# jiexray/gelly-streaming

Measured on AMD Instinct MI355X. Metric: edges/sec (whole node) for streaming CC on RMAT-26, higher is better.
Workload: dtype int64; 1 GPU; rmat26-cc-stream; scale=26, edges=1073741824, micro_batch=1048576, combine_every_edges_per_gpu=4194304, combine=none at 1 GPU (same cadence), ids=sparse 64-bit (scrambled), capacity_hint=33554432, vertices_labelled=32802821, parallelism=single GPU

## Files before the change

gelly-streaming_amd/__init__.py:

```python
import ctypes
import os

import numpy as np


_HERE = os.path.dirname(os.path.abspath(__file__))
LIB_PATH = os.path.join(_HERE, "lib", "libgs_summary.so")
if os.environ.get("GS_LIB_VARIANT"):
    LIB_PATH = os.path.join(_HERE, "lib_" + os.environ["GS_LIB_VARIANT"], "libgs_summary.so")

KIND_CC = 0
KIND_SIGNED = 1
KIND_DEGREE = 2

DEGREE_ALL = 0
DEGREE_IN = 1
DEGREE_OUT = 2

GS_OK = 0
GS_ERR_INVALID = -1
GS_ERR_HIP = -2
GS_ERR_CAPACITY = -3
GS_ERR_TRUNCATED = -4
GS_ERR_PARSE = -5

SEP_WHITESPACE = 0
SEP_TAB = 1

KERNEL_IDS = {"fold": 0, "stage": 1, "export": 2, "init": 3}

EXPORTED_SYMBOLS = (
    "gs_last_error", "gs_version", "gs_create", "gs_destroy", "gs_reset", "gs_fold", "gs_fold_device",
    "gs_combine", "gs_sync", "gs_num_vertices", "gs_find", "gs_export_labels", "gs_export_labels_device",
    "gs_bip_status", "gs_export_colouring", "gs_serialize", "gs_deserialize", "gs_set_delta_tracking",
    "gs_take_delta_records", "gs_fold_take_device", "gs_delta_stage", "gs_fold_records_device", "gs_fold_exchange_device",
    "gs_get_stream", "gs_set_pipelining", "gs_set_hot_index", "gs_hot_index_stats", "gs_set_profiling", "gs_kernel_stats", "gs_table_capacity", "gs_counters", "gs_debug_counters",
    "gs_gen_rmat", "gs_gen_er", "gs_gen_bip",
    "gs_parse_edges_device", "gs_fold_text", "gs_parse_set_profiling", "gs_parse_profile", "gs_parse_release",
    "gs_group_unique_id", "gs_group_create", "gs_group_fold_device", "gs_group_finish", "gs_group_stats",
    "gs_group_destroy", "gs_group_tree_combine", "gs_combine_exported_device",
    "gs_group_fold_batches_device", "gs_group_set_ramp", "gs_export_labels_part_device",
    "gs_delta_capacity", "gs_find_labels_device", "gs_capacity_stats",
    "gs_set_change_tracking", "gs_take_changes_device", "gs_take_changes",
    "gs_fold_records_counted_device", "gs_reset_config", "gs_wait_event", "gs_wait_stream", "gs_fold_device_after",
    "gs_fold_parity", "gs_set_window_server", "gs_window_server_stats", "gs_set_batch_dedup",
    "gs_digest", "gs_group_comm_ranks", "gs_group_set_phase_timing", "gs_group_phase_stats",
    "gs_group_set_comm_api", "gs_testing_set", "gs_testing_get", "gs_testing_group_forest", "gs_hbm_bytes", "gs_create_bytes",
    "gs_group_create_partitioned", "gs_group_part_fold_device", "gs_group_part_combine",
    "gs_group_part_labels_device", "gs_group_part_status", "gs_group_part_reset", "gs_group_part_stats",
    "gs_group_part_phase_stats",
    "gs_num_components", "gs_export_components_device", "gs_export_components",
    "gs_degree_fold", "gs_degree_fold_device", "gs_degree_find_device", "gs_degree_export_device",
    "gs_degree_export", "gs_degree_distribution_device", "gs_degree_distribution",
    "gs_triangle_create", "gs_triangle_destroy", "gs_triangle_reset", "gs_triangle_fold", "gs_triangle_fold_device",
    "gs_triangle_count", "gs_triangle_count_device", "gs_triangle_find_device", "gs_triangle_export_device",
    "gs_triangle_export", "gs_triangle_sync", "gs_triangle_get_stream", "gs_triangle_wait_stream",
    "gs_testing_triangle_stats", "gs_testing_triangle_bins",
    "gs_slice_create", "gs_slice_destroy", "gs_slice_window", "gs_slice_window_device", "gs_slice_size",
    "gs_slice_reduce_device", "gs_slice_reduce", "gs_slice_neighborhoods_device", "gs_slice_neighborhoods",
    "gs_slice_sync", "gs_slice_get_stream", "gs_slice_wait_stream", "gs_testing_slice_stats",
    "gs_distinct_create", "gs_distinct_destroy", "gs_distinct_reset", "gs_distinct_fold", "gs_distinct_fold_device",
    "gs_distinct_size", "gs_distinct_new_edges_device", "gs_distinct_new_edges", "gs_distinct_new_vertices_device",
    "gs_distinct_new_vertices", "gs_distinct_vertices_device", "gs_distinct_vertices", "gs_distinct_edges_device",
    "gs_distinct_edges", "gs_distinct_rank_device", "gs_distinct_contains_device", "gs_distinct_sync",
    "gs_distinct_get_stream", "gs_distinct_wait_stream", "gs_testing_distinct_stats",
    "gs_testing_distinct_phases",
    "gs_spanner_create", "gs_spanner_destroy", "gs_spanner_reset", "gs_spanner_fold", "gs_spanner_fold_device",
    "gs_spanner_add", "gs_spanner_within", "gs_spanner_within_device", "gs_spanner_combine", "gs_spanner_count",
    "gs_spanner_export_device", "gs_spanner_export", "gs_spanner_neighbors", "gs_spanner_sync",
# ... 122 lines not shown
    L.gs_window_server_stats.argtypes = [_vp, ctypes.POINTER(_u64), ctypes.POINTER(_u64)]
    L.gs_fold_device.argtypes = [_vp, _vp, _vp, _vp, _sz, _sz]
    L.gs_fold_device_after.argtypes = [_vp, _vp, _vp, _vp, _sz, _sz, _vp]
    L.gs_wait_event.argtypes = [_vp, _vp]
    L.gs_wait_stream.argtypes = [_vp, _vp]
    L.gs_combine.argtypes = [_vp, _vp]
    L.gs_sync.argtypes = [_vp]
    L.gs_num_vertices.argtypes = [_vp, ctypes.POINTER(_u64)]
    L.gs_find.argtypes = [_vp, _i64, ctypes.POINTER(_i64), ctypes.POINTER(ctypes.c_int)]
    L.gs_export_labels.argtypes = [_vp, _vp, _vp, _sz, ctypes.POINTER(_sz)]
    L.gs_export_labels_device.argtypes = [_vp, _vp, _vp, _vp, _sz, ctypes.POINTER(_sz)]
    L.gs_bip_status.argtypes = [_vp, ctypes.POINTER(ctypes.c_int)]
    L.gs_export_colouring.argtypes = [_vp, _vp, _vp, _vp, _sz, ctypes.POINTER(_sz)]
    L.gs_serialize.argtypes = [_vp, _vp, _sz, ctypes.POINTER(_sz)]
    L.gs_deserialize.argtypes = [_vp, _vp, _sz]
    L.gs_set_delta_tracking.argtypes = [_vp, ctypes.c_int]
    L.gs_take_delta_records.argtypes = [_vp, _vp, _sz, _vp]
    L.gs_fold_take_device.argtypes = [_vp, _vp, _vp, _sz, _vp, _sz, _vp, _vp]
    L.gs_fold_records_device.argtypes = [_vp, _vp, _sz, ctypes.c_int]
    L.gs_fold_records_counted_device.argtypes = [_vp, _vp, _sz, _vp, ctypes.c_int]
    L.gs_delta_stage.argtypes = [_vp, _vp, _sz, ctypes.c_int, _vp]
    L.gs_fold_exchange_device.argtypes = [_vp, _vp, _vp, _sz, _sz, ctypes.c_int, ctypes.c_int]
    L.gs_delta_capacity.argtypes = [_vp, ctypes.POINTER(_u64)]
    L.gs_find_labels_device.argtypes = [_vp, _vp, _sz, _vp, _vp]
    L.gs_capacity_stats.argtypes = [_vp, ctypes.POINTER(_u64), ctypes.POINTER(_u64), ctypes.POINTER(ctypes.c_double)]
    L.gs_set_change_tracking.argtypes = [_vp, ctypes.c_int]
    L.gs_take_changes_device.argtypes = [_vp, _vp, _vp, _vp, _sz, ctypes.POINTER(_u64)]
    L.gs_take_changes.argtypes = [_vp, _vp, _vp, _vp, _sz, ctypes.POINTER(_u64)]
    L.gs_get_stream.argtypes = [_vp, ctypes.POINTER(_vp)]
    L.gs_set_profiling.argtypes = [_vp, ctypes.c_int]
    L.gs_set_pipelining.argtypes = [_vp, ctypes.c_int]
    L.gs_set_hot_index.argtypes = [_vp, ctypes.c_int, _u64, ctypes.c_uint32]
    L.gs_hot_index_stats.argtypes = [_vp, ctypes.POINTER(_u64)]
    L.gs_kernel_stats.argtypes = [_vp, ctypes.c_int, ctypes.POINTER(_u64), ctypes.POINTER(ctypes.c_double)]
    L.gs_table_capacity.argtypes = [_vp, ctypes.POINTER(_u64)]
    L.gs_counters.argtypes = [_vp, ctypes.POINTER(_u64)]
    L.gs_debug_counters.argtypes = [_vp, ctypes.POINTER(_u64), ctypes.c_int]
    L.gs_gen_rmat.argtypes = [_vp, _vp, _vp, _u64, _u64, ctypes.c_int, _u64, ctypes.c_int]
    L.gs_gen_er.argtypes = [_vp, _vp, _vp, _u64, _u64, ctypes.c_int, _u64, ctypes.c_int]
    L.gs_gen_bip.argtypes = [_vp, _vp, _vp, _u64, _u64, ctypes.c_int, _u64, _vp, _sz]
    L.gs_parse_edges_device.argtypes = [_vp, _vp, _sz, ctypes.c_int, _vp, _vp, _sz, ctypes.POINTER(_u64),
                                        ctypes.POINTER(_i64)]
    L.gs_parse_set_profiling.argtypes = [ctypes.c_int]
    L.gs_parse_profile.argtypes = [ctypes.POINTER(ctypes.c_double), ctypes.POINTER(_u64)]
    L.gs_fold_text.argtypes = [_vp, ctypes.c_char_p, _sz, ctypes.c_int, ctypes.POINTER(_u64), ctypes.POINTER(_i64)]
    L.gs_group_unique_id.argtypes = [_vp]
    L.gs_group_create.argtypes = [ctypes.POINTER(_vp), _vp, _vp, ctypes.c_int, ctypes.c_int, _sz]
    L.gs_group_fold_device.argtypes = [_vp, _vp, _vp, _sz]
    L.gs_group_finish.argtypes = [_vp]
    L.gs_group_stats.argtypes = [_vp, ctypes.POINTER(_u64), ctypes.POINTER(_u64), ctypes.POINTER(_u64)]
    L.gs_group_destroy.argtypes = [_vp]
    L.gs_group_tree_combine.argtypes = [_vp]
    L.gs_group_fold_batches_device.argtypes = [_vp, _vp, _vp, _sz, _sz]
    L.gs_group_set_ramp.argtypes = [_vp, _sz, _sz]
    L.gs_export_labels_part_device.argtypes = [_vp, ctypes.c_int, ctypes.c_int, _vp, _vp, _vp, _sz,
                                               ctypes.POINTER(_sz)]
    L.gs_combine_exported_device.argtypes = [_vp, _vp, _vp, _vp, _sz, ctypes.c_int]
    L.gs_digest.argtypes = [_vp, ctypes.POINTER(_u64)]
    L.gs_group_comm_ranks.argtypes = [_vp, ctypes.POINTER(ctypes.c_int), ctypes.POINTER(ctypes.c_int)]
    L.gs_group_set_phase_timing.argtypes = [_vp, ctypes.c_int]
    L.gs_group_phase_stats.argtypes = [_vp, ctypes.POINTER(ctypes.c_double)]
    L.gs_group_set_comm_api.argtypes = [_vp]
    L.gs_group_create_partitioned.argtypes = [ctypes.POINTER(_vp), _vp, _vp, ctypes.c_int, ctypes.c_int, _u64, _sz]
    L.gs_group_part_fold_device.argtypes = [_vp, _vp, _vp, _sz]
    L.gs_group_part_combine.argtypes = [_vp]
    L.gs_group_part_labels_device.argtypes = [_vp, _vp, _vp, _vp, _sz, ctypes.POINTER(_sz)]
# ... 170 lines not shown


def digest_rows(v, label, parity=None):
    import torch

    def srl(x, k):
        return (x >> k) & ((1 << (64 - k)) - 1)

    def mix(z):
        z = (z ^ srl(z, 30)) * -4658895280553007687
        z = (z ^ srl(z, 27)) * -7723592293110705685
        return z ^ srl(z, 31)
    if v.numel() == 0:
        return 0
    a = mix(v ^ 0x243F6A8885A308D3)
    b = mix(label + (parity.to(torch.int64) * 0x13198A2E03707344 if parity is not None else 0))
    return int(torch.sum(a * b).item()) & ((1 << 64) - 1)


TESTING_KNOBS = {"server_idle_us": 0, "changes_walk_max": 1, "parse_lb_timeout_us": 2, "group_self_apply": 3,
                 "group_data_lag": 4, "degree_variant": 5, "triangle_variant": 6, "triangle_profile": 7,
                 "slice_profile": 8, "distinct_profile": 9, "spanner_round_cap": 10, "spanner_lds_set": 11,
                 "spanner_arenas": 12}


def testing_set(knob, value):
    _check(lib().gs_testing_set(TESTING_KNOBS[knob], -1 if value is None else int(value)))


def testing_get(knob):
    return lib().gs_testing_get(TESTING_KNOBS[knob])


class testing:

    def __init__(self, **knobs):
        self.knobs = knobs

    def __enter__(self):
        for k, v in self.knobs.items():
            testing_set(k, v)
        return self

    def __exit__(self, *a):
        for k in self.knobs:
            testing_set(k, None)


FAKE_COMM_PATH = os.path.join(_HERE, "host", "bin", "libgs_fakecomm.so")
_fake = None


def fake_comm():
    global _fake
    if _fake is None:
        lib()
        if not os.path.exists(FAKE_COMM_PATH):
            raise ImportError("libgs_fakecomm.so not built (%s); run __graft_entry__.build()" % FAKE_COMM_PATH)
        F = ctypes.CDLL(FAKE_COMM_PATH)
        F.gs_fake_comm_api.restype = _vp
        F.gs_fake_comm_last_error.restype = ctypes.c_int
        F.gs_fake_comm_order_hash.restype = _u64
        _fake = F
    return _fake


# ... 1409 lines not shown
```

gelly-streaming_amd/csrc/gs_capi.cpp:

```cpp
#include <hip/hip_runtime.h>

#include <algorithm>
#include <atomic>
#include <chrono>
#include <mutex>
#include <unordered_map>
#include <cstdio>
#include <cstring>
#include <string>
#include <thread>
#include <vector>

#include "gs_ingest.h"
#include "gs_internal.hpp"

#ifndef GS_YOUNG_HEAD_LOG2
#define GS_YOUNG_HEAD_LOG2 14
#endif

namespace gsi {

thread_local std::string g_err;

int fail(int code, const std::string& msg) {
// ... 92 lines not shown
  if (h->x_v) {
    if (int rc = wait_x_consumer(h)) return rc;
    GS_HIP(hipStreamSynchronize(h->stream));
  }
  h->x_cap = 0;
  const uint64_t c = std::max<uint64_t>(rows, (uint64_t)(kMaxLoad * (double)h->cap) + 2);
  GS_HIP(h->x_v.alloc(c));
  GS_HIP(h->x_l.alloc(c));
  GS_HIP(h->x_p.alloc(c));
  h->x_cap = c;
  return GS_OK;
}

void reset_capacity_tracking(gs_summary* h, uint64_t nv) {
  h->rep_epoch++;
  h->nv_ub = nv;
  h->nv_exact = nv;
  h->e_exact = 0;
  h->e_launched = 0;
  h->e_lost = 0;
  for (int i = 0; i < gs_summary::kRepStreams; ++i) h->rep_skip[i] = 0, h->rep_pending[i] = 0;
  h->rep_pending_edges = 0;
}

#ifndef GS_HOT_LOG2
#define GS_HOT_LOG2 17
#endif
#ifndef GS_HOT_REFRESH_EVERY
#define GS_HOT_REFRESH_EVERY 16
#endif
#ifndef GS_HOT_SAMPLE_LOG2
#define GS_HOT_SAMPLE_LOG2 20
#endif
constexpr int kHotLog2 = GS_HOT_LOG2;
constexpr int kHotMaxLog2 = 20;
constexpr uint64_t kHotFirstEdges = 1ull << 26;
constexpr uint32_t kHotEvery = 2048;
constexpr uint32_t kHotRefreshEvery = GS_HOT_REFRESH_EVERY;
constexpr uint32_t kHotRefreshPerBuild = 16;
constexpr uint64_t kHotMinTableBytes = 256ull << 20;
constexpr size_t kHotSampleEdges = 1u << GS_HOT_SAMPLE_LOG2;

int hot_log2(const gs_summary* h) {
  if (h->kind != GS_KIND_CC || h->hot_cfg < 0) return 0;
  if (h->track || h->changes || h->srv_on || h->side || h->group_lanes) return 0;
  if (h->hot_cfg > 0) return h->hot_cfg;
  if (h->cap * sizeof(gs::Slot) < kHotMinTableBytes) return 0;
  return kHotLog2;
}

void hot_drop(gs_summary* h) {
  h->hot_live = -1;
  h->hot_building = -1;
  h->hot_read_on[0] = h->hot_read_on[1] = false;
  h->hot_edges = 0;
  h->hot_folds = 0;
  h->hot_folds_r = 0;
}

int hot_before_fold(gs_summary* h) {
  if (h->hot_building < 0 || hipEventQuery(h->hot_built) != hipSuccess) return GS_OK;
  const int old = h->hot_live;
  h->hot_live = h->hot_building;
  h->hot_building = -1;
  if (old < 0) return GS_OK;
  for (int i = 0; i <= gs_summary::kLanes; ++i) {
    hipStream_t st = i < gs_summary::kLanes ? (hipStream_t)h->lane[i] : (hipStream_t)h->stream;
    if (i < gs_summary::kLanes && !h->lane[i]) continue;
    GS_HIP(hipEventRecord(h->hot_read[old][i], st));
  }
  h->hot_read_on[old] = true;
  return GS_OK;
}

int hot_after_fold(gs_summary* h, const int64_t* src, const int64_t* dst, size_t c, size_t stride, hipStream_t st,
                   int hl) {
  h->hot_edges += c;
  h->hot_folds++;
  h->hot_folds_r++;
  if (h->hot_building >= 0) return GS_OK;
  const uint64_t first = h->hot_cfg ? h->hot_first : kHotFirstEdges;
  const uint32_t every = h->hot_cfg ? h->hot_every : kHotEvery;
  const bool build = h->hot_live < 0 ? h->hot_edges >= first : h->hot_folds >= every;
  const uint32_t refresh_every = h->hot_cfg ? every / kHotRefreshPerBuild : kHotRefreshEvery;
  if (!build) {
    if (!(h->hot_live >= 0 && refresh_every && h->hot_folds_r >= refresh_every)) return GS_OK;
    h->hot_refreshes++;
    h->hot_folds_r = 0;
    GS_LAUNCH(gs::launch_hot_refresh(h->table(), h->hot_buf[h->hot_live], hl, st));
    return GS_OK;
  }
  if (h->hot_alloc_log2 != hl) {
    h->hot_alloc_log2 = 0;
    for (auto& b : h->hot_buf) GS_HIP(b.alloc(gs::hot_buckets(hl) + 1));
    GS_HIP(h->hot_scratch.alloc(gs::hot_scratch_words(hl)));
    if (!h->hot_built) {
      GS_HIP(h->hot_built.create());
      for (auto& r : h->hot_read)
        for (Event& e : r) GS_HIP(e.create());
    }
    h->hot_alloc_log2 = hl;
  }
  const int b = h->hot_live < 0 ? 0 : h->hot_live ^ 1;
  if (h->hot_read_on[b]) {
    for (int i = 0; i <= gs_summary::kLanes; ++i)
      if (i == gs_summary::kLanes || h->lane[i]) GS_HIP(hipStreamWaitEvent(st, h->hot_read[b][i], 0));
    h->hot_read_on[b] = false;
  }
  h->hot_folds = 0;
  h->hot_builds++;
  GS_LAUNCH(gs::launch_hot_build(h->table(), src, dst, (uint32_t)std::min(c, kHotSampleEdges), (uint32_t)stride,
                                 h->hot_buf[b], hl, h->hot_scratch, st));
  GS_HIP(hipEventRecord(h->hot_built, st));
  h->hot_building = b;
  h->hot_folds_r = 0;
  return GS_OK;
}

}

uint64_t create_capacity(uint64_t capacity_hint) {
  const uint64_t cap = next_pow2(std::max<uint64_t>(kSlotsPerHintedVertex * std::max<uint64_t>(capacity_hint, 1), 1024));
  return std::min(cap, kMaxCap);
}

uint64_t create_bytes(uint64_t cap) {
  return (cap + 1) * sizeof(gs::Slot) + (uint64_t)gs::kShards * (cap / gs::kShards + 1024) * 4 +
         (uint64_t)gs::CTR_COUNT * gs::kCtrStride * 4 + 64;
}

namespace {

int alloc_vlist(gs_summary* h) {
  h->vshard_cap = (uint32_t)(h->cap / gs::kShards + 1024);
  GS_HIP(h->vlist.alloc((uint64_t)gs::kShards * h->vshard_cap));
  return GS_OK;
}

int alloc_table(gs_summary* h, uint64_t cap, bool keep_delta = false) {
  h->cap = cap;
  h->logcap = log2_ceil(cap);
  GS_HIP(h->tab.alloc(cap + 1));
  if (int rc = alloc_vlist(h)) return rc;
  memset(h->h_flags, 0, 16);
  hot_drop(h);
// ... 1507 lines not shown
  if (int rc = join_lanes(h)) return rc;
  GS_HIP(hipStreamSynchronize(h->stream));
  hot_drop(h);
  if (h->hot_alloc_log2 != (log2_entries > 0 ? log2_entries : kHotLog2)) {
    h->hot_alloc_log2 = 0;
    for (auto& b : h->hot_buf) b.reset();
    h->hot_scratch.reset();
  }
  h->hot_cfg = log2_entries < 0 ? -1 : log2_entries;
  h->hot_first = first_after_edges;
  h->hot_every = rebuild_every_folds;
  return GS_OK;
}

int gs_hot_index_stats(gs_handle h, uint64_t* out4) {
  if (int rc = check_any(h)) return rc;
  if (!out4) return fail(GS_ERR_INVALID, "out is null");
  DeviceGuard g(h->device);
  if (int rc = join_lanes(h)) return rc;
  GS_HIP(hipStreamSynchronize(h->stream));
  if (int rc = hot_before_fold(h)) return rc;
  out4[0] = h->hot_builds;
  out4[1] = 0;
  out4[2] = h->hot_live >= 0 ? (uint64_t)h->hot_alloc_log2 : 0;
  out4[3] = h->hot_refreshes;
  if (h->hot_live >= 0) {
    std::vector<gs::HotBucket> e(gs::hot_buckets(h->hot_alloc_log2));
    GS_HIP(hipMemcpy(e.data(), h->hot_buf[h->hot_live], e.size() * sizeof(gs::HotBucket), hipMemcpyDeviceToHost));
    for (const gs::HotBucket& x : e) out4[1] += (x.key[0] != gs::kEmpty) + (x.key[1] != gs::kEmpty);
  }
  return GS_OK;
}

int gs_table_capacity(gs_handle h, uint64_t* slots) {
  if (int rc = check_any(h)) return rc;
  if (!slots) return fail(GS_ERR_INVALID, "slots is null");
  *slots = h->cap;
  return GS_OK;
}

}

namespace gsi {

int x_scratch(gs_summary* h, uint64_t rows) {
  if (int rc = ensure_x(h, rows)) return rc;
  return wait_x_consumer(h);
}

void exact_count(gs_summary* h, uint64_t nv) { note_exact_count(h, nv); }

int rebuild_table(gs_summary* h, uint64_t cap) { return alloc_table(h, cap, true); }

int comp_staging(gs_summary* h, uint64_t nv, uint64_t nc) { return ensure_comp_staging(h, nv, nc); }
int dev_stage(gs_summary* h, size_t edges) { return ensure_dev_stage(h, edges); }

}

extern "C" int gs_testing_set(int knob, int64_t value) {
  if (knob < 0 || knob >= GS_TESTING_KNOBS) return gsi::fail(GS_ERR_INVALID, "unknown test knob");
  gsi::g_testing[knob].store(value < 0 ? -1 : value, std::memory_order_relaxed);
  return GS_OK;
}

extern "C" int64_t gs_testing_get(int knob) {
  if (knob < 0 || knob >= GS_TESTING_KNOBS) return -1;
// ... 19 lines not shown
```

gelly-streaming_amd/csrc/gs_hot_k.hip:

```cpp
#include "gs_kernels.hpp"

namespace gs {

namespace {

constexpr int kHotSketchLog2 = 4;
constexpr uint32_t kHotBS = 256;
constexpr uint32_t kVoteCells = 1024;
constexpr uint32_t kVoteEvery = 8;
constexpr int kVoteRounds = 8;

__device__ __forceinline__ uint32_t sketch_pos(int64_t key, int log2_ids) {
  return (uint32_t)(((uint64_t)key * 0xC2B2AE3D27D4EB4Full) >> (64 - kHotSketchLog2 - log2_ids));
}
__device__ __forceinline__ unsigned long long hot_rank(uint32_t count, int64_t key) {
  return ((unsigned long long)count << 32) | (uint32_t)(((uint64_t)key * 0x9E3779B97F4A7C15ull) >> 32);
}

__device__ __forceinline__ bool wave_combine(int64_t key, bool has, uint32_t* elect, uint32_t* dups, uint32_t& cnt) {
  const uint32_t lane = threadIdx.x & 63u;
  const uint32_t e = (uint32_t)(((uint64_t)key * 0x9E3779B97F4A7C15ull) >> 57);
  __syncthreads();
  dups[lane] = 0;
  if (has) elect[e] = lane;
  __syncthreads();
  const uint32_t w = has ? elect[e] : lane;
  const int64_t kw = __shfl(key, (int)w, 64);
  const bool dup = has && w != lane && kw == key;
  if (dup) atomicAdd(&dups[w], 1u);
  __syncthreads();
  cnt = 1u + dups[lane];
  return has && !dup;
}

struct HotSample {
  const int64_t* src;
  const int64_t* dst;
  uint32_t n, stride;
};

struct HotScratch {
  unsigned long long* best1;
  unsigned long long* best2;
  unsigned long long* vote;
  uint32_t* cells;
  uint32_t* slot1;
  uint32_t* sketch;
  int64_t* keys;
  uint32_t* root;
};
__host__ __device__ inline uint64_t scratch_zeroed_words(int log2_ids) {
  const uint64_t ids = 1ull << log2_ids;
  return ids  + 1 + kVoteCells / 2 + (ids + 1) / 2 + ((ids << kHotSketchLog2) >> 1);
}
inline HotScratch scratch_of(unsigned long long* w, int log2_ids) {
  const uint64_t ids = 1ull << log2_ids, buckets = ids >> 1;
  HotScratch s;
  s.best1 = w;
  s.best2 = s.best1 + buckets;
  s.vote = s.best2 + buckets;
  s.cells = reinterpret_cast<uint32_t*>(s.vote + 1);
  s.slot1 = s.cells + kVoteCells;
  s.sketch = s.slot1 + ids;
  s.keys = reinterpret_cast<int64_t*>(w + scratch_zeroed_words(log2_ids));
  s.root = reinterpret_cast<uint32_t*>(s.keys + ids);
  return s;
}

__device__ __forceinline__ bool sample_key(const HotSample& s, int j, int64_t& key) {
  const uint32_t i = blockIdx.x * kHotBS + threadIdx.x;
  key = 0;
  if (i >= s.n) return false;
  key = (j ? s.dst : s.src)[(size_t)i * s.stride];
  return key != kEmpty;
}

__global__ __launch_bounds__(kHotBS) void k_hot_count(HotSample s, uint32_t* sketch, int log2_ids) {
  __shared__ uint32_t elect[kHotBS / 64][128], dups[kHotBS / 64][64];
  const uint32_t wv = threadIdx.x >> 6;
#pragma unroll
  for (int j = 0; j < 2; ++j) {
    int64_t key;
    uint32_t cnt;
    const bool has = sample_key(s, j, key);
    if (wave_combine(key, has, elect[wv], dups[wv], cnt)) atomicAdd(&sketch[sketch_pos(key, log2_ids)], cnt);
  }
}

__global__ __launch_bounds__(kHotBS) void k_hot_select(HotSample s, HotScratch x, int log2_ids) {
  __shared__ uint32_t elect[kHotBS / 64][128], dups[kHotBS / 64][64];
  const uint32_t wv = threadIdx.x >> 6;
#pragma unroll
  for (int j = 0; j < 2; ++j) {
    int64_t key;
    uint32_t cnt;
    const bool has = sample_key(s, j, key);
    if (!wave_combine(key, has, elect[wv], dups[wv], cnt)) continue;
    const unsigned long long r = hot_rank(x.sketch[sketch_pos(key, log2_ids)], key);
    const uint32_t p = hot_pos(key, 65 - log2_ids);
    const unsigned long long seen = x.best1[p];
    if (seen == r) continue;
    unsigned long long lower = r;
    if (seen < r) {
      const unsigned long long old = atomicMax(x.best1 + p, r);
      if (old == r) continue;
      lower = old < r ? old : r;
    }
    if (lower && x.best2[p] < lower) atomicMax(x.best2 + p, lower);
  }
}

__global__ __launch_bounds__(kHotBS) void k_hot_claim(Table t, HotSample s, HotScratch x, int log2_ids) {
  __shared__ uint32_t elect[kHotBS / 64][128], dups[kHotBS / 64][64];
  const uint32_t wv = threadIdx.x >> 6;
#pragma unroll
  for (int j = 0; j < 2; ++j) {
    int64_t key;
    uint32_t cnt;
    const bool has = sample_key(s, j, key);
    if (!wave_combine(key, has, elect[wv], dups[wv], cnt)) continue;
    const unsigned long long r = hot_rank(x.sketch[sketch_pos(key, log2_ids)], key);
    const uint32_t p = hot_pos(key, 65 - log2_ids);
    const bool second = x.best1[p] != r;
    unsigned long long* b = (second ? x.best2 : x.best1) + p;
    if (*b != r || atomicCAS(b, r, 0ull) != r) continue;
    uint32_t link = 0;
    const uint32_t slot = lookup_find(t, key, link);
    if (slot == kNoSlot) continue;
    x.keys[2 * p + second] = key;
    x.slot1[2 * p + second] = slot + 1;
  }
}

__global__ __launch_bounds__(kHotBS) void k_hot_root(Table t, HotScratch x, uint32_t ids) {
  const uint32_t i = blockIdx.x * kHotBS + threadIdx.x;
  uint32_t root = kNoSlot;
  if (i < ids && x.slot1[i]) {
    const uint32_t slot = x.slot1[i] - 1;
    int64_t k = 0;
    uint32_t l = 0, par = 0;
    load_slot(t.tab + slot, k, l);
    root = find_ro(t, slot, l, k, par);
    x.root[i] = root;
  }
  if (gridDim.x > 8 * kVoteEvery && blockIdx.x % kVoteEvery) return;
  const int lane = (int)(threadIdx.x & 63u);
  bool pend = root != kNoSlot;
  for (int round = 0; round < kVoteRounds; ++round) {
    const unsigned long long m = __ballot(pend);
    if (!m) break;
    const int leader = __ffsll((long long)m) - 1;
    const uint32_t r0 = (uint32_t)__shfl((int)root, leader, 64);
    const bool same = pend && root == r0;
    const uint32_t n = (uint32_t)__popcll(__ballot(same));
    if (lane == leader) {
      const uint32_t c = atomicAdd(&x.cells[(r0 * 0x9E3779B1u) >> 22], n) + n;
      atomicMax(x.vote, ((unsigned long long)c << 32) | r0);
    }
    if (same) pend = false;
  }
}

__global__ __launch_bounds__(kHotBS) void k_hot_place(HotScratch x, HotBucket* out, uint32_t buckets) {
  const uint32_t p = blockIdx.x * kHotBS + threadIdx.x;
  if (p >= buckets) return;
  const unsigned long long v = *x.vote;
  const uint32_t g = v ? (uint32_t)v : kNoSlot;
  const bool h0 = x.slot1[2 * p] && x.root[2 * p] == g, h1 = x.slot1[2 * p + 1] && x.root[2 * p + 1] == g;
  const uint64_t k0 = (uint64_t)(h0 ? x.keys[2 * p] : kEmpty), k1 = (uint64_t)(h1 ? x.keys[2 * p + 1] : kEmpty);
  *reinterpret_cast<uint4*>(out + p) =
      make_uint4((uint32_t)k0, (uint32_t)(k0 >> 32), (uint32_t)k1, (uint32_t)(k1 >> 32));
  if (p == 0) *reinterpret_cast<uint4*>(out + buckets) = make_uint4(g, g, 0u, 0u);
}

__global__ __launch_bounds__(64) void k_hot_refresh(Table t, HotHeader* h) {
  if (threadIdx.x) return;
  const uint32_t g = h->g;
  if (g == kNoSlot) return;
  int64_t k = 0;
  uint32_t l = 0, par = 0;
  load_slot(t.tab + g, k, l);
  h->g2 = find_ro(t, g, l, k, par);
}

}

uint64_t hot_scratch_words(int log2_ids) {
  const uint64_t ids = 1ull << log2_ids;
  return scratch_zeroed_words(log2_ids) + ids + (ids + 1) / 2;
}

void launch_hot_build(const Table& t, const int64_t* src, const int64_t* dst, uint32_t n, uint32_t stride,
                      HotBucket* out, int log2_ids, unsigned long long* scratch, hipStream_t st) {
  const uint32_t ids = 1u << log2_ids, buckets = (uint32_t)hot_buckets(log2_ids);
  const HotScratch x = scratch_of(scratch, log2_ids);
  (void)hipMemsetAsync(scratch, 0, scratch_zeroed_words(log2_ids) * 8, st);
  const HotSample s{src, dst, n, stride};
  const dim3 g((n + kHotBS - 1) / kHotBS), b(kHotBS);
  hipLaunchKernelGGL(k_hot_count, g, b, 0, st, s, x.sketch, log2_ids);
  hipLaunchKernelGGL(k_hot_select, g, b, 0, st, s, x, log2_ids);
  hipLaunchKernelGGL(k_hot_claim, g, b, 0, st, t, s, x, log2_ids);
  hipLaunchKernelGGL(k_hot_root, dim3((ids + kHotBS - 1) / kHotBS), b, 0, st, t, x, ids);
  hipLaunchKernelGGL(k_hot_place, dim3((buckets + kHotBS - 1) / kHotBS), b, 0, st, x, out, buckets);
}

void launch_hot_refresh(const Table& t, HotBucket* live, int log2_ids, hipStream_t st) {
  hipLaunchKernelGGL(k_hot_refresh, dim3(1), dim3(64), 0, st, t, reinterpret_cast<HotHeader*>(live + hot_buckets(log2_ids)));
}

}
```

gelly-streaming_amd/csrc/gs_internal.hpp:

```cpp
#pragma once
#include <hip/hip_runtime.h>

#include <string>
#include <vector>

#include "gs_devbuf.hpp"
#include "gs_grow.hpp"
#include "gs_ingest.hpp"
#include "gs_kernels.hpp"
#include "gs_own.hpp"
#include "gs_sort.hpp"
#include "gs_summary.h"
#include "gs_testing.h"

namespace gsi {

int fail(int code, const std::string& msg);
int64_t testing_value(int knob, int64_t product);

constexpr int kMaxDevices = 64;
uint64_t create_capacity(uint64_t capacity_hint);
uint64_t create_bytes(uint64_t cap);

#define GS_HIP(call)                                                                                  \
// ... 267 lines not shown
  gsi::DevBuf<int64_t> co_member;
  gsi::DevBuf<uint8_t> co_sign;
  uint64_t co_vcap = 0, co_ccap = 0;
  uint64_t deg_total = 0;
  gsi::TextIngest text;
  int pipe_depth = 1;
  uint64_t api_calls = 0;
  int group_lanes = 0;
  static constexpr int kLanes = 4;
  gsi::Lane lane[kLanes];
  gsi::Event main_ev;
  gsi::Event idle_ev;
  bool xwait = false;
  int lane_next = 0;
  int last_lane = -1;
  bool lanes_dirty = false;
  bool export_ctr_zero = false;
  int hot_cfg = 0;
  uint64_t hot_first = 0;
  uint32_t hot_every = 0;
  gsi::DevBuf<gs::HotBucket> hot_buf[2];
  gsi::DevBuf<unsigned long long> hot_scratch;
  int hot_alloc_log2 = 0;
  int hot_live = -1;
  int hot_building = -1;
  gsi::Event hot_built;
  gsi::Event hot_read[2][kLanes + 1];
  bool hot_read_on[2] = {false, false};
  uint64_t hot_edges = 0;
  uint32_t hot_folds = 0;
  uint32_t hot_folds_r = 0;
  uint64_t hot_builds = 0;
  uint64_t hot_refreshes = 0;
  hipStream_t side = nullptr;
  hipEvent_t side_ev = nullptr;
  bool side_dirty = false;
  bool dedup = false;
  static constexpr int kDedupSets = kLanes + 2;
  gsi::DevBuf<unsigned long long> dd_tab[kDedupSets];
  gsi::DevBuf<uint8_t> dd_w[kDedupSets];
  uint64_t dd_edges[kDedupSets] = {};
  uint64_t dd_kept_hint = 0;
  bool srv_on = false, srv_running = false;
  int srv_fits = -1;
  gsi::WindowServer srv;
  unsigned long long srv_seq = 0;
  uint64_t srv_launches = 0, srv_windows = 0;
  bool profiling = false;
  gsi::SpanTimer spans;
  uint64_t launches[gsi::KID_N] = {0, 0, 0, 0};
  double total_ms[gsi::KID_N] = {0, 0, 0, 0};

  gs::Table table() const {
    gs::Table t = gsi::make_table(tab, ctr, cap, logcap);
    t.vlist = vlist;
    t.vshard_cap = vshard_cap;
    t.mark_new = changes ? 1 : 0;
    t.hflags = h_flags.dev();
    return t;
  }
  gs::Delta delta(int set = -1) const {
    if (set < 0) set = dset;
    gs::Delta D;
    D.drec = drec ? drec + (size_t)set * gs::kShards * delta_shard_cap * 3 : nullptr;
    D.shard_cap = delta_shard_cap;
    D.dctr = (uint32_t)(gs::CTR_DELTA + set * gs::kShards);
// ... 56 lines not shown
```

gelly-streaming_amd/csrc/gs_kernels.hpp:

```cpp
#pragma once
#include <hip/hip_runtime.h>
#include <stdint.h>

#include "gs_device.hpp"

namespace gs {

struct FoldLaunch {
  const int64_t* src = nullptr;
  const int64_t* dst = nullptr;
  const uint8_t* w = nullptr;
  uint32_t n = 0;
  uint32_t stride = 1;
  uint32_t w_stride = 1;
  uint32_t rows = 0;
  int skip_rank = -1;
  const unsigned long long* counts = nullptr;
  uint32_t base = 0;
  const unsigned long long* n_dev = nullptr;
  const uint32_t* fail_in = nullptr;
  uint32_t shard0 = 0;
  int64_t* take_out = nullptr;
  unsigned long long take_cap = 0;
  unsigned long long* take_count = nullptr;
// ... 25 lines not shown
  unsigned long long taken;
  unsigned long long bc_init;
  unsigned long long pad[5];
};
struct alignas(64) ServerBcast {
  unsigned long long seq, src, dst, n, rec, cap, cnt, done_seq;
};
void launch_window_server(bool sign, const Table& t, const Delta& D, ServerBox* box, ServerBcast* bc,
                          unsigned long long* done, unsigned long long seq0, unsigned long long idle_ticks,
                          hipStream_t st);
int window_server_resident_blocks(bool sign, int device);

void launch_init(Slot* tab, uint64_t nslots, hipStream_t st, uint32_t* ctr = nullptr);
void launch_dedup(const int64_t* src, const int64_t* dst, uint32_t n, unsigned long long* tab, uint32_t mask,
                  uint8_t* w, hipStream_t st);
void launch_reset_list(const Table& t, uint32_t* nxt, uint64_t bound, hipStream_t st);
void launch_fold(bool sign, bool track, const Table& t, const Delta& D, const FoldLaunch& f, hipStream_t st);
void launch_export(const Table& t, int64_t* ov, int64_t* ol, uint8_t* op, uint64_t cap_out, hipStream_t st,
                   int part = 0, int nparts = 1, bool by_list = false);
void launch_export_list(const Table& t, int64_t* ov, int64_t* ol, uint8_t* op, uint64_t cap_out, uint64_t bound,
                        hipStream_t st);
void launch_digest(const Table& t, unsigned long long* out, uint64_t bound, hipStream_t st);
void launch_stage(const Table& t, const Delta& D, int64_t* out, uint64_t cap, int width,
                  unsigned long long* count_out, bool with_fail, hipStream_t st);
void launch_report(uint32_t* ctr, uint64_t n, unsigned long long* out, unsigned epoch, hipStream_t st);
void launch_headers(const unsigned long long* counts, int nranks, long long* out, long long seq, hipStream_t st);
constexpr unsigned long long kSignalFlagBit = 1ull << 62;
void launch_signal(unsigned long long* out, unsigned long long seq, const uint32_t* vals, int nvals, int stride,
                   hipStream_t st, bool clear = false, const uint32_t* flag = nullptr);
void launch_find_one(const Table& t, int64_t key, int64_t* out, hipStream_t st);
void launch_find_batch(const Table& t, const int64_t* v, uint64_t n, int64_t* label, uint8_t* found, uint8_t* parity,
                       hipStream_t st);

inline uint64_t hot_buckets(int log2_ids) { return 1ull << (log2_ids - 1); }
uint64_t hot_scratch_words(int log2_ids);
void launch_hot_build(const Table& t, const int64_t* src, const int64_t* dst, uint32_t n, uint32_t stride,
                      HotBucket* out, int log2_ids, unsigned long long* scratch, hipStream_t st);
void launch_hot_refresh(const Table& t, HotBucket* live, int log2_ids, hipStream_t st);

void launch_iota(uint32_t* nxt, uint64_t n, hipStream_t st);
void launch_relist(const Table& t, uint32_t* nxt, hipStream_t st);
void launch_emit_records(const Table& t, uint32_t* nxt, const int64_t* rec, const unsigned long long* nrec,
                         uint64_t nrec_bound, uint32_t walk_max, int64_t* ov, int64_t* ol, uint8_t* op, uint64_t cap,
                         uint32_t* big, hipStream_t st);
void launch_emit_scan(const Table& t, int64_t* ov, int64_t* ol, uint8_t* op, uint64_t cap, bool all, hipStream_t st);
void launch_clear_big(const Table& t, const uint32_t* big, uint64_t n, hipStream_t st);
void launch_emit_new(const Table& t, uint32_t* vmark, int64_t* ov, int64_t* ol, uint8_t* op, uint64_t cap,
                     uint64_t bound, bool emit, hipStream_t st);

}
```

include/gs_testing.h:

```cpp
#ifndef GS_TESTING_H
#define GS_TESTING_H

#include <stdint.h>

#ifdef __cplusplus
extern "C" {
#endif

enum gs_testing_knob {
  GS_TESTING_SERVER_IDLE_US = 0,
  GS_TESTING_CHANGES_WALK_MAX = 1,
  GS_TESTING_PARSE_LB_TIMEOUT_US = 2,
  GS_TESTING_GROUP_SELF_APPLY = 3,
  GS_TESTING_GROUP_DATA_LAG = 4,
  GS_TESTING_DEGREE_VARIANT = 5,
  GS_TESTING_TRIANGLE_VARIANT = 6,
  GS_TESTING_TRIANGLE_PROFILE = 7,
  GS_TESTING_SLICE_PROFILE = 8,
  GS_TESTING_DISTINCT_PROFILE = 9,
  GS_TESTING_SPANNER_ROUND_CAP = 10,
  GS_TESTING_SPANNER_LDS_SET = 11,
  GS_TESTING_SPANNER_ARENAS = 12,
  GS_TESTING_KNOBS = 13
};
// ... 4 lines not shown

int gs_testing_group_forest(void* g, void** forest);

int gs_testing_triangle_stats(void* t, uint64_t* out);

int gs_testing_triangle_bins(void* t, uint64_t* out);

int gs_testing_slice_stats(void* s, uint64_t* out);

int gs_testing_distinct_stats(void* d, uint64_t* out);

int gs_testing_distinct_phases(void* d, uint64_t* out);

int gs_testing_spanner_stats(void* s, uint64_t* out);

int gs_testing_spanner_generation(void* s, int64_t set, uint64_t* out);

int gs_testing_matching_stats(void* m, uint64_t* out);

int gs_testing_matching_tune(void* m, int what, int64_t value);

int gs_testing_trisample_stats(void* t, uint64_t* out);

int gs_testing_trisample_tune(void* t, int what, int64_t value);

int gs_testing_degstream_stats(void* d, uint64_t* out);

int gs_testing_degstream_tune(void* d, int what, int64_t value);

int gs_testing_tristream_stats(void* d, uint64_t* out);

int gs_testing_tristream_tune(void* d, int what, int64_t value);

#ifdef __cplusplus
}
#endif
#endif
```

Before: 29.94 billion edges/s.

## Widen hot-index sketch and accumulate counts across multiple sampled folds

The hot-vertex index build now takes its heavy-hitter sketch counts over several micro-batches (two by default) before selecting hot keys, and the sketch grows from 2^4 to 2^6 counters per id, with an optional second row for count-min estimation. The aim is to pick truly hot vertices more accurately, so that more fold lookups hit the hot index and skip the main table. In exchange there is extra zeroing and counting work, larger scratch memory, and index rebuilds that lag by one fold. Testing hooks are added to tune these parameters and to read back the chosen keys.

```diff
diff --git a/gelly-streaming_amd/__init__.py b/gelly-streaming_amd/__init__.py
--- a/gelly-streaming_amd/__init__.py
+++ b/gelly-streaming_amd/__init__.py
@@ -34,7 +34,7 @@
     "gs_combine", "gs_sync", "gs_num_vertices", "gs_find", "gs_export_labels", "gs_export_labels_device",
     "gs_bip_status", "gs_export_colouring", "gs_serialize", "gs_deserialize", "gs_set_delta_tracking",
     "gs_take_delta_records", "gs_fold_take_device", "gs_delta_stage", "gs_fold_records_device", "gs_fold_exchange_device",
-    "gs_get_stream", "gs_set_pipelining", "gs_set_hot_index", "gs_hot_index_stats", "gs_set_profiling", "gs_kernel_stats", "gs_table_capacity", "gs_counters", "gs_debug_counters",
+    "gs_get_stream", "gs_set_pipelining", "gs_set_hot_index", "gs_hot_index_stats", "gs_testing_hot_tune", "gs_testing_hot_keys", "gs_set_profiling", "gs_kernel_stats", "gs_table_capacity", "gs_counters", "gs_debug_counters",
     "gs_gen_rmat", "gs_gen_er", "gs_gen_bip",
     "gs_parse_edges_device", "gs_fold_text", "gs_parse_set_profiling", "gs_parse_profile", "gs_parse_release",
     "gs_group_unique_id", "gs_group_create", "gs_group_fold_device", "gs_group_finish", "gs_group_stats",
@@ -223,6 +223,10 @@
     L.gs_set_pipelining.argtypes = [_vp, ctypes.c_int]
     L.gs_set_hot_index.argtypes = [_vp, ctypes.c_int, _u64, ctypes.c_uint32]
     L.gs_hot_index_stats.argtypes = [_vp, ctypes.POINTER(_u64)]
+    if hasattr(L, "gs_testing_hot_tune"):
+        L.gs_testing_hot_tune.argtypes = [_vp, ctypes.c_int, ctypes.c_int64]
+        L.gs_testing_hot_keys.argtypes = [_vp, ctypes.POINTER(_i64), _u64]
+        L.gs_testing_hot_keys.restype = _i64
     L.gs_kernel_stats.argtypes = [_vp, ctypes.c_int, ctypes.POINTER(_u64), ctypes.POINTER(ctypes.c_double)]
     L.gs_table_capacity.argtypes = [_vp, ctypes.POINTER(_u64)]
     L.gs_counters.argtypes = [_vp, ctypes.POINTER(_u64)]
@@ -459,6 +463,24 @@
     return lib().gs_testing_get(TESTING_KNOBS[knob])
 
 
+def testing_hot_tune(summary, rows=None, sketch_log2=None, sample_folds=None):
+    for what, v in enumerate((rows, sketch_log2, sample_folds)):
+        if v is not None:
+            _check(lib().gs_testing_hot_tune(summary._h, what, int(v)))
+
+
+def testing_hot_keys(summary):
+    import numpy as np
+    n = lib().gs_testing_hot_keys(summary._h, None, 0)
+    if n < 0:
+        _check(int(n))
+    out = (_i64 * max(int(n), 1))()
+    m = lib().gs_testing_hot_keys(summary._h, out, int(n))
+    if m < 0:
+        _check(int(m))
+    return np.frombuffer(out, dtype=np.int64, count=int(min(n, m))).copy()
+
+
 class testing:
 
     def __init__(self, **knobs):
diff --git a/gelly-streaming_amd/csrc/gs_capi.cpp b/gelly-streaming_amd/csrc/gs_capi.cpp
--- a/gelly-streaming_amd/csrc/gs_capi.cpp
+++ b/gelly-streaming_amd/csrc/gs_capi.cpp
@@ -148,6 +148,18 @@
 #ifndef GS_HOT_SAMPLE_LOG2
 #define GS_HOT_SAMPLE_LOG2 20
 #endif
+#ifndef GS_HOT_SKETCH_ROWS
+#define GS_HOT_SKETCH_ROWS 1
+#endif
+#ifndef GS_HOT_SKETCH_LOG2
+#define GS_HOT_SKETCH_LOG2 6
+#endif
+#ifndef GS_HOT_SAMPLE_FOLDS
+#define GS_HOT_SAMPLE_FOLDS 2
+#endif
+static_assert(GS_HOT_SKETCH_ROWS == 1 || GS_HOT_SKETCH_ROWS == 2, "GS_HOT_SKETCH_ROWS");
+static_assert(GS_HOT_SKETCH_LOG2 >= 0 && GS_HOT_SKETCH_LOG2 <= 6, "GS_HOT_SKETCH_LOG2");
+static_assert(GS_HOT_SAMPLE_FOLDS == 1 || GS_HOT_SAMPLE_FOLDS == 2 || GS_HOT_SAMPLE_FOLDS == 4, "GS_HOT_SAMPLE_FOLDS");
 constexpr int kHotLog2 = GS_HOT_LOG2;
 constexpr int kHotMaxLog2 = 20;
 constexpr uint64_t kHotFirstEdges = 1ull << 26;
@@ -157,6 +169,14 @@
 constexpr uint64_t kHotMinTableBytes = 256ull << 20;
 constexpr size_t kHotSampleEdges = 1u << GS_HOT_SAMPLE_LOG2;
 
+gs::HotTune hot_tune(const gs_summary* h) {
+  return gs::HotTune{h->hot_rows ? h->hot_rows : GS_HOT_SKETCH_ROWS,
+                     h->hot_sketch_log2 >= 0 ? h->hot_sketch_log2 : GS_HOT_SKETCH_LOG2};
+}
+uint32_t hot_sample_folds(const gs_summary* h) {
+  return h->hot_sample_folds ? h->hot_sample_folds : (h->hot_cfg ? 1u : (uint32_t)GS_HOT_SAMPLE_FOLDS);
+}
+
 int hot_log2(const gs_summary* h) {
   if (h->kind != GS_KIND_CC || h->hot_cfg < 0) return 0;
   if (h->track || h->changes || h->srv_on || h->side || h->group_lanes) return 0;
@@ -172,6 +192,7 @@
   h->hot_edges = 0;
   h->hot_folds = 0;
   h->hot_folds_r = 0;
+  h->hot_counted = 0;
 }
 
 int hot_before_fold(gs_summary* h) {
@@ -206,17 +227,35 @@
     GS_LAUNCH(gs::launch_hot_refresh(h->table(), h->hot_buf[h->hot_live], hl, st));
     return GS_OK;
   }
+  const gs::HotTune tune = hot_tune(h);
   if (h->hot_alloc_log2 != hl) {
     h->hot_alloc_log2 = 0;
     for (auto& b : h->hot_buf) GS_HIP(b.alloc(gs::hot_buckets(hl) + 1));
-    GS_HIP(h->hot_scratch.alloc(gs::hot_scratch_words(hl)));
+    GS_HIP(h->hot_scratch.alloc(gs::hot_scratch_words(hl, tune)));
     if (!h->hot_built) {
       GS_HIP(h->hot_built.create());
+      GS_HIP(h->hot_zeroed.create());
+      for (Event& e : h->hot_count_ev) GS_HIP(e.create());
       for (auto& r : h->hot_read)
         for (Event& e : r) GS_HIP(e.create());
     }
     h->hot_alloc_log2 = hl;
   }
+  const uint32_t n = (uint32_t)std::min(c, kHotSampleEdges);
+  if (h->hot_counted == 0) {
+    GS_LAUNCH(gs::launch_hot_zero(hl, tune, h->hot_scratch, st));
+    GS_HIP(hipEventRecord(h->hot_zeroed, st));
+  } else {
+    GS_HIP(hipStreamWaitEvent(st, h->hot_zeroed, 0));
+  }
+  if (h->hot_counted + 1 < hot_sample_folds(h)) {
+    GS_LAUNCH(gs::launch_hot_count(src, dst, n, (uint32_t)stride, hl, tune, h->hot_scratch, st));
+    GS_HIP(hipEventRecord(h->hot_count_ev[h->hot_counted], st));
+    h->hot_counted++;
+    return GS_OK;
+  }
+  for (uint32_t i = 0; i < h->hot_counted; ++i) GS_HIP(hipStreamWaitEvent(st, h->hot_count_ev[i], 0));
+  h->hot_counted = 0;
   const int b = h->hot_live < 0 ? 0 : h->hot_live ^ 1;
   if (h->hot_read_on[b]) {
     for (int i = 0; i <= gs_summary::kLanes; ++i)
@@ -225,8 +264,7 @@
   }
   h->hot_folds = 0;
   h->hot_builds++;
-  GS_LAUNCH(gs::launch_hot_build(h->table(), src, dst, (uint32_t)std::min(c, kHotSampleEdges), (uint32_t)stride,
-                                 h->hot_buf[b], hl, h->hot_scratch, st));
+  GS_LAUNCH(gs::launch_hot_build(h->table(), src, dst, n, (uint32_t)stride, h->hot_buf[b], hl, tune, h->hot_scratch, st));
   GS_HIP(hipEventRecord(h->hot_built, st));
   h->hot_building = b;
   h->hot_folds_r = 0;
@@ -1800,6 +1838,50 @@
   return GS_OK;
 }
 
+int gs_testing_hot_tune(void* hv, int what, int64_t value) {
+  gs_handle h = static_cast<gs_handle>(hv);
+  if (int rc = check_any(h)) return rc;
+  if (h->kind != GS_KIND_CC) return fail(GS_ERR_INVALID, "the hot index serves connected-components summaries only");
+  if (what < 0 || what > 2) return fail(GS_ERR_INVALID, "hot tune: what is 0, 1 or 2");
+  if (value >= 0) {
+    if (what == 0 && value != 1 && value != 2) return fail(GS_ERR_INVALID, "hot tune: 1 or 2 sketch rows");
+    if (what == 1 && value > 6) return fail(GS_ERR_INVALID, "hot tune: at most 2^6 counters per id");
+    if (what == 2 && value != 1 && value != 2 && value != 4) return fail(GS_ERR_INVALID, "hot tune: 1, 2 or 4 sample folds");
+  }
+  DeviceGuard g(h->device);
+  if (int rc = join_lanes(h)) return rc;
+  GS_HIP(hipStreamSynchronize(h->stream));
+  hot_drop(h);
+  h->hot_alloc_log2 = 0;
+  for (auto& b : h->hot_buf) b.reset();
+  h->hot_scratch.reset();
+  if (what == 0) h->hot_rows = value < 0 ? 0 : (int)value;
+  if (what == 1) h->hot_sketch_log2 = value < 0 ? -1 : (int)value;
+  if (what == 2) h->hot_sample_folds = value < 0 ? 0u : (uint32_t)value;
+  return GS_OK;
+}
+
+int64_t gs_testing_hot_keys(void* hv, int64_t* out, uint64_t cap) {
+  gs_handle h = static_cast<gs_handle>(hv);
+  if (int rc = check_any(h)) return rc;
+  if (!out && cap) return fail(GS_ERR_INVALID, "out is null");
+  DeviceGuard g(h->device);
+  if (int rc = join_lanes(h)) return rc;
+  GS_HIP(hipStreamSynchronize(h->stream));
+  if (int rc = hot_before_fold(h)) return rc;
+  if (h->hot_live < 0) return 0;
+  std::vector<gs::HotBucket> e(gs::hot_buckets(h->hot_alloc_log2));
+  GS_HIP(hipMemcpy(e.data(), h->hot_buf[h->hot_live], e.size() * sizeof(gs::HotBucket), hipMemcpyDeviceToHost));
+  uint64_t n = 0;
+  for (const gs::HotBucket& x : e)
+    for (int64_t k : x.key)
+      if (k != gs::kEmpty) {
+        if (n < cap) out[n] = k;
+        ++n;
+      }
+  return (int64_t)n;
+}
+
 int gs_table_capacity(gs_handle h, uint64_t* slots) {
   if (int rc = check_any(h)) return rc;
   if (!slots) return fail(GS_ERR_INVALID, "slots is null");
diff --git a/gelly-streaming_amd/csrc/gs_hot_k.hip b/gelly-streaming_amd/csrc/gs_hot_k.hip
--- a/gelly-streaming_amd/csrc/gs_hot_k.hip
+++ b/gelly-streaming_amd/csrc/gs_hot_k.hip
@@ -4,14 +4,23 @@
 
 namespace {
 
-constexpr int kHotSketchLog2 = 4;
 constexpr uint32_t kHotBS = 256;
 constexpr uint32_t kVoteCells = 1024;
 constexpr uint32_t kVoteEvery = 8;
 constexpr int kVoteRounds = 8;
 
-__device__ __forceinline__ uint32_t sketch_pos(int64_t key, int log2_ids) {
-  return (uint32_t)(((uint64_t)key * 0xC2B2AE3D27D4EB4Full) >> (64 - kHotSketchLog2 - log2_ids));
+struct HotSketch {
+  uint32_t* c;
+  int rows, bits;
+};
+__device__ __forceinline__ uint32_t sketch_pos(int64_t key, int row, int bits) {
+  const uint64_t mul = row ? 0xA24BAED4963EE407ull : 0xC2B2AE3D27D4EB4Full;
+  return ((uint32_t)row << bits) + (uint32_t)(((uint64_t)key * mul) >> (64 - bits));
+}
+__device__ __forceinline__ uint32_t sketch_count(const HotSketch& k, int64_t key) {
+  uint32_t c = k.c[sketch_pos(key, 0, k.bits)];
+  if (k.rows > 1) c = min(c, k.c[sketch_pos(key, 1, k.bits)]);
+  return c;
 }
 __device__ __forceinline__ unsigned long long hot_rank(uint32_t count, int64_t key) {
   return ((unsigned long long)count << 32) | (uint32_t)(((uint64_t)key * 0x9E3779B97F4A7C15ull) >> 32);
@@ -45,15 +54,16 @@
   unsigned long long* vote;
   uint32_t* cells;
   uint32_t* slot1;
-  uint32_t* sketch;
+  HotSketch sketch;
   int64_t* keys;
   uint32_t* root;
 };
-__host__ __device__ inline uint64_t scratch_zeroed_words(int log2_ids) {
+inline uint64_t scratch_zeroed_words(int log2_ids, const HotTune& tune) {
   const uint64_t ids = 1ull << log2_ids;
-  return ids  + 1 + kVoteCells / 2 + (ids + 1) / 2 + ((ids << kHotSketchLog2) >> 1);
-}
-inline HotScratch scratch_of(unsigned long long* w, int log2_ids) {
+  return ids  + 1 + kVoteCells / 2 + (ids + 1) / 2 +
+         (((uint64_t)tune.rows << (tune.sketch_log2 + log2_ids)) + 1) / 2;
+}
+inline HotScratch scratch_of(unsigned long long* w, int log2_ids, const HotTune& tune) {
   const uint64_t ids = 1ull << log2_ids, buckets = ids >> 1;
   HotScratch s;
   s.best1 = w;
@@ -61,8 +71,8 @@
   s.vote = s.best2 + buckets;
   s.cells = reinterpret_cast<uint32_t*>(s.vote + 1);
   s.slot1 = s.cells + kVoteCells;
-  s.sketch = s.slot1 + ids;
-  s.keys = reinterpret_cast<int64_t*>(w + scratch_zeroed_words(log2_ids));
+  s.sketch = HotSketch{s.slot1 + ids, tune.rows, tune.sketch_log2 + log2_ids};
+  s.keys = reinterpret_cast<int64_t*>(w + scratch_zeroed_words(log2_ids, tune));
   s.root = reinterpret_cast<uint32_t*>(s.keys + ids);
   return s;
 }
@@ -75,7 +85,7 @@
   return key != kEmpty;
 }
 
-__global__ __launch_bounds__(kHotBS) void k_hot_count(HotSample s, uint32_t* sketch, int log2_ids) {
+__global__ __launch_bounds__(kHotBS) void k_hot_count(HotSample s, HotSketch sketch) {
   __shared__ uint32_t elect[kHotBS / 64][128], dups[kHotBS / 64][64];
   const uint32_t wv = threadIdx.x >> 6;
 #pragma unroll
@@ -83,7 +93,8 @@
     int64_t key;
     uint32_t cnt;
     const bool has = sample_key(s, j, key);
-    if (wave_combine(key, has, elect[wv], dups[wv], cnt)) atomicAdd(&sketch[sketch_pos(key, log2_ids)], cnt);
+    if (!wave_combine(key, has, elect[wv], dups[wv], cnt)) continue;
+    for (int row = 0; row < sketch.rows; ++row) atomicAdd(&sketch.c[sketch_pos(key, row, sketch.bits)], cnt);
   }
 }
 
@@ -96,7 +107,7 @@
     uint32_t cnt;
     const bool has = sample_key(s, j, key);
     if (!wave_combine(key, has, elect[wv], dups[wv], cnt)) continue;
-    const unsigned long long r = hot_rank(x.sketch[sketch_pos(key, log2_ids)], key);
+    const unsigned long long r = hot_rank(sketch_count(x.sketch, key), key);
     const uint32_t p = hot_pos(key, 65 - log2_ids);
     const unsigned long long seen = x.best1[p];
     if (seen == r) continue;
@@ -119,7 +130,7 @@
     uint32_t cnt;
     const bool has = sample_key(s, j, key);
     if (!wave_combine(key, has, elect[wv], dups[wv], cnt)) continue;
-    const unsigned long long r = hot_rank(x.sketch[sketch_pos(key, log2_ids)], key);
+    const unsigned long long r = hot_rank(sketch_count(x.sketch, key), key);
     const uint32_t p = hot_pos(key, 65 - log2_ids);
     const bool second = x.best1[p] != r;
     unsigned long long* b = (second ? x.best2 : x.best1) + p;
@@ -185,19 +196,30 @@
 
 }
 
-uint64_t hot_scratch_words(int log2_ids) {
+uint64_t hot_scratch_words(int log2_ids, const HotTune& tune) {
   const uint64_t ids = 1ull << log2_ids;
-  return scratch_zeroed_words(log2_ids) + ids + (ids + 1) / 2;
+  return scratch_zeroed_words(log2_ids, tune) + ids + (ids + 1) / 2;
+}
+
+void launch_hot_zero(int log2_ids, const HotTune& tune, unsigned long long* scratch, hipStream_t st) {
+  (void)hipMemsetAsync(scratch, 0, scratch_zeroed_words(log2_ids, tune) * 8, st);
+}
+
+void launch_hot_count(const int64_t* src, const int64_t* dst, uint32_t n, uint32_t stride, int log2_ids,
+                      const HotTune& tune, unsigned long long* scratch, hipStream_t st) {
+  if (!n) return;
+  const HotScratch x = scratch_of(scratch, log2_ids, tune);
+  const HotSample s{src, dst, n, stride};
+  hipLaunchKernelGGL(k_hot_count, dim3((n + kHotBS - 1) / kHotBS), dim3(kHotBS), 0, st, s, x.sketch);
 }
 
 void launch_hot_build(const Table& t, const int64_t* src, const int64_t* dst, uint32_t n, uint32_t stride,
-                      HotBucket* out, int log2_ids, unsigned long long* scratch, hipStream_t st) {
+                      HotBucket* out, int log2_ids, const HotTune& tune, unsigned long long* scratch, hipStream_t st) {
   const uint32_t ids = 1u << log2_ids, buckets = (uint32_t)hot_buckets(log2_ids);
-  const HotScratch x = scratch_of(scratch, log2_ids);
-  (void)hipMemsetAsync(scratch, 0, scratch_zeroed_words(log2_ids) * 8, st);
+  const HotScratch x = scratch_of(scratch, log2_ids, tune);
   const HotSample s{src, dst, n, stride};
   const dim3 g((n + kHotBS - 1) / kHotBS), b(kHotBS);
-  hipLaunchKernelGGL(k_hot_count, g, b, 0, st, s, x.sketch, log2_ids);
+  hipLaunchKernelGGL(k_hot_count, g, b, 0, st, s, x.sketch);
   hipLaunchKernelGGL(k_hot_select, g, b, 0, st, s, x, log2_ids);
   hipLaunchKernelGGL(k_hot_claim, g, b, 0, st, t, s, x, log2_ids);
   hipLaunchKernelGGL(k_hot_root, dim3((ids + kHotBS - 1) / kHotBS), b, 0, st, t, x, ids);
diff --git a/gelly-streaming_amd/csrc/gs_internal.hpp b/gelly-streaming_amd/csrc/gs_internal.hpp
--- a/gelly-streaming_amd/csrc/gs_internal.hpp
+++ b/gelly-streaming_amd/csrc/gs_internal.hpp
@@ -323,6 +323,11 @@
   uint32_t hot_folds_r = 0;
   uint64_t hot_builds = 0;
   uint64_t hot_refreshes = 0;
+  int hot_rows = 0, hot_sketch_log2 = -1;
+  uint32_t hot_sample_folds = 0;
+  uint32_t hot_counted = 0;
+  gsi::Event hot_zeroed;
+  gsi::Event hot_count_ev[3];
   hipStream_t side = nullptr;
   hipEvent_t side_ev = nullptr;
   bool side_dirty = false;
diff --git a/gelly-streaming_amd/csrc/gs_kernels.hpp b/gelly-streaming_amd/csrc/gs_kernels.hpp
--- a/gelly-streaming_amd/csrc/gs_kernels.hpp
+++ b/gelly-streaming_amd/csrc/gs_kernels.hpp
@@ -81,10 +81,17 @@
 void launch_find_batch(const Table& t, const int64_t* v, uint64_t n, int64_t* label, uint8_t* found, uint8_t* parity,
                        hipStream_t st);
 
+struct HotTune {
+  int rows;
+  int sketch_log2;
+};
 inline uint64_t hot_buckets(int log2_ids) { return 1ull << (log2_ids - 1); }
-uint64_t hot_scratch_words(int log2_ids);
+uint64_t hot_scratch_words(int log2_ids, const HotTune& tune);
+void launch_hot_zero(int log2_ids, const HotTune& tune, unsigned long long* scratch, hipStream_t st);
+void launch_hot_count(const int64_t* src, const int64_t* dst, uint32_t n, uint32_t stride, int log2_ids,
+                      const HotTune& tune, unsigned long long* scratch, hipStream_t st);
 void launch_hot_build(const Table& t, const int64_t* src, const int64_t* dst, uint32_t n, uint32_t stride,
-                      HotBucket* out, int log2_ids, unsigned long long* scratch, hipStream_t st);
+                      HotBucket* out, int log2_ids, const HotTune& tune, unsigned long long* scratch, hipStream_t st);
 void launch_hot_refresh(const Table& t, HotBucket* live, int log2_ids, hipStream_t st);
 
 void launch_iota(uint32_t* nxt, uint64_t n, hipStream_t st);
diff --git a/include/gs_testing.h b/include/gs_testing.h
--- a/include/gs_testing.h
+++ b/include/gs_testing.h
@@ -60,6 +60,10 @@
 
 int gs_testing_tristream_tune(void* d, int what, int64_t value);
 
+int gs_testing_hot_tune(void* h, int what, int64_t value);
+
+int64_t gs_testing_hot_keys(void* h, int64_t* out, uint64_t cap);
+
 #ifdef __cplusplus
 }
 #endif
```

Measured after the change: 30.53 billion edges/s, median of 6. 2.0% higher.
